# sebasv/lp

Measured on NVIDIA B200. Metric: ipm_iterations_per_s, higher is better.
Workload: dtype f64

## Files before the change

### lp_b200/csrc/cholesky.cu

```cuda
#include <nccl.h>

#include <algorithm>
#include <cstring>
#include <mutex>
#include <type_traits>

#include "dist_schedule.hpp"
#include "kernels.hpp"
#include "panel_factor.cuh"

namespace lpb {

namespace {

constexpr int NB = 128;
constexpr int LDS = NB + 1;
constexpr int TRSM_ROWS = 64;

__global__ void __launch_bounds__(512)
potf2_kernel(double* __restrict__ Mat, int64_t ldm, int k0, int nb, int* __restrict__ info) {
  extern __shared__ double S[];
  double* diag = S + NB * LDS;
  const int tx = threadIdx.x, ty = threadIdx.y, tid = ty * 32 + tx;
  double* blk = Mat + (int64_t)k0 * ldm + k0;
  for (int i = ty; i < nb; i += 16)
    for (int k = tx; k <= i; k += 32) S[i * LDS + k] = blk[(int64_t)i * ldm + k];
  __syncthreads();

  for (int j = 0; j < nb; ++j) {
    const double ajj = S[j * LDS + j];
    if (!(ajj > 0.0) || !isfinite(ajj)) {
      if (tid == 0 && *info == 0) *info = k0 + j + 1;
      for (int i = j + tid; i < nb; i += 512) diag[i] = __longlong_as_double(0x7ff8000000000000ll);
      break;
    }
    const double d = sqrt(ajj);
    if (tid == 0) diag[j] = d;
    if (tid < nb - j - 1) S[(j + 1 + tid) * LDS + j] /= d;
    __syncthreads();
    for (int i = j + 1 + ty; i < nb; i += 16) {
      const double lij = S[i * LDS + j];
      for (int k = j + 1 + tx; k <= i; k += 32) S[i * LDS + k] -= lij * S[k * LDS + j];
    }
    __syncthreads();
  }
  __syncthreads();
  for (int i = ty; i < nb; i += 16)
    for (int k = tx; k <= i; k += 32) blk[(int64_t)i * ldm + k] = (k == i) ? diag[i] : S[i * LDS + k];
}

constexpr int SB = 16;
constexpr int NSB = NB / SB;
constexpr int XDP = SB + 1;
constexpr int TWP = 9;

__device__ __forceinline__ void complete_block_inverse(double* S, const double* rdiag, double* Tw, int tid) {
  const int lane = tid & 31, warp = tid >> 5;
  const int b = warp >> 1, h = warp & 1;
  const int ii = lane & 15, cg = lane >> 4;
  double* tw = Tw + warp * SB * TWP;
  for (int d = 1; d < NSB; ++d) {
    if (b < NSB - d) {
      const int j = b, i = b + d;
      const int ccb = 8 * h + 4 * cg;
      double acc[4] = {0.0, 0.0, 0.0, 0.0};
      const double* lrow = S + (i * SB + ii) * LDS;
#pragma unroll
      for (int l = 0; l < SB; ++l) {
        const double lv = lrow[j * SB + l];
#pragma unroll
        for (int e = 0; e < 4; ++e) {
          const int cc = ccb + e;
          const double up = S[(j * SB + cc) * LDS + j * SB + l];
          const double xv = (l > cc) ? up : ((l == cc) ? rdiag[j * SB + cc] : 0.0);
          acc[e] += lv * xv;
        }
      }
      for (int k = j + 1; k < i; ++k) {
#pragma unroll
        for (int l = 0; l < SB; ++l) {
          const double lv = lrow[k * SB + l];
#pragma unroll
          for (int e = 0; e < 4; ++e) acc[e] += lv * S[(j * SB + ccb + e) * LDS + k * SB + l];
        }
      }
#pragma unroll
      for (int e = 0; e < 4; ++e) tw[ii * TWP + 4 * cg + e] = acc[e];
      __syncwarp();
      double o[4] = {0.0, 0.0, 0.0, 0.0};
#pragma unroll
// ... 1295 lines not shown
int set_smem(K kern, size_t bytes) {
  LPB_CUDA(cudaFuncSetAttribute(kern, cudaFuncAttributeMaxDynamicSharedMemorySize, (int)bytes));
  return LPB_OK;
}

constexpr size_t kPotf2Smem = (size_t)(NB * LDS + NB) * sizeof(double);
constexpr size_t kPotf2InvSmem = (size_t)(NB * LDS + NB + 2 * SB * XDP + 16 * SB * TWP + panel_factor_scratch(XDP)) * sizeof(double);
constexpr size_t kTrsmSmem = (size_t)((NB + TRSM_ROWS) * LDS) * sizeof(double);
constexpr size_t kTrsvSmem = (size_t)(NB * LDS + NB + 2 * NB) * sizeof(double);

int configure_once() {
  static PerDeviceOnce once;
  return once.run([](int) -> int {
  LPB_TRY(set_smem(potf2_kernel, kPotf2Smem));
  LPB_TRY(set_smem(potf2_inv_kernel, kPotf2InvSmem));
  LPB_TRY(set_smem(trsm_kernel, kTrsmSmem));
  LPB_TRY(set_smem(trsm_blocked_kernel, kTrsmBlockedSmem));
  LPB_TRY(set_smem(trsm_dmma_blocked_kernel, kTrsmDmmaSmem));
  LPB_TRY(set_smem(trsv_diag_kernel<false, 1>, kTrsvSmem));
  LPB_TRY(set_smem(trsv_diag_kernel<false, 2>, kTrsvSmem));
  LPB_TRY(set_smem(trsv_diag_kernel<true, 1>, kTrsvSmem));
  LPB_TRY(set_smem(trsv_diag_kernel<true, 2>, kTrsvSmem));
  return LPB_OK;
  });
}

#define LPB_KCHECK(lc)             \
  do {                             \
    (lc).launches++;               \
    LPB_CUDA(cudaGetLastError());  \
  } while (0)

}

struct CholWs {
  int64_t nblk, ldy, off_y, off_flags, off_wt, off_xt, total;
  explicit CholWs(int64_t m) {
    nblk = ceil_div(m, NB);
    ldy = round_up(m, 2);
    off_y = nblk * NB * NB;
    off_flags = off_y + 2 * ldy;
    off_wt = off_flags + round_up(nblk, 2);
    off_xt = off_wt + nblk * 2 * NB * 2;
    total = off_xt + nblk * 2 * NB * 2;
  }
};

static int ensure_chol_ws(LaunchCtx& lc, int64_t m) {
  const int64_t need = CholWs(m).total;
  if (lc.chol_ws_cap >= need) return LPB_OK;
  if (lc.chol_ws) cudaFree(lc.chol_ws);
  lc.chol_ws = nullptr;
  lc.chol_ws_cap = 0;
  lc.linv_valid_m = -1;
  void* p = nullptr;
  LPB_CUDA(cudaMalloc(&p, sizeof(double) * (size_t)need));
  LPB_CUDA(cudaMemsetAsync(p, 0, sizeof(double) * (size_t)need, lc.stream));
  lc.chol_ws = static_cast<double*>(p);
  lc.chol_ws_cap = need;
  return LPB_OK;
}

static int finish_factor(LaunchCtx& lc, int64_t m, double* Mat, int64_t ldm) {
  if (lc.potf2_impl == 1) {
    lc.linv_valid_m = -1;
    lc.linv_mat = nullptr;
    return LPB_OK;
  }
  if (!lc.linv_full) {
    static PerDeviceOnce once;
    LPB_TRY(once.run([](int) -> int { return set_smem(linv_complete_kernel, kLinvCompleteSmem); }));
    linv_complete_kernel<<<(unsigned)ceil_div(m, NB), dim3(32, 16), kLinvCompleteSmem, lc.stream>>>(Mat, ldm, m, lc.chol_ws);
    LPB_KCHECK(lc);
    lc.linv_full = true;
  }
  lc.linv_valid_m = m;
  lc.linv_mat = Mat;
  return LPB_OK;
}

static int k_potrf_dist(LaunchCtx& lc, int64_t m, double* Mat, int64_t ldm);
static int k_potrf_dist2(LaunchCtx& lc, int64_t m, double* Mat, int64_t ldm);

static int k_potrf_lookahead(LaunchCtx& lc, int64_t m, double* Mat, int64_t ldm) {
  if (!lc.side_stream) {
    int lo = 0, hi = 0;
    LPB_CUDA(cudaDeviceGetStreamPriorityRange(&lo, &hi));
    LPB_CUDA(cudaStreamCreateWithPriority(&lc.side_stream, cudaStreamNonBlocking, hi));
    for (int e = 0; e < 2; ++e) {
      LPB_CUDA(cudaEventCreateWithFlags(&lc.ev_col[e], cudaEventDisableTiming));
      LPB_CUDA(cudaEventCreateWithFlags(&lc.ev_pan[e], cudaEventDisableTiming));
    }
  }
  const int T = (int)ceil_div(m, NB);
  lc.linv_full = false;
  auto nb_of = [&](int k) { return (int)((m - (int64_t)k * NB) < NB ? (m - (int64_t)k * NB) : NB); };
  auto potf2 = [&](int k, cudaStream_t st) -> int {
    potf2_inv_kernel<<<1, dim3(32, 16), kPotf2InvSmem, st>>>(Mat, ldm, k * NB, nb_of(k), lc.info_dev,
                                                             lc.chol_ws + (int64_t)k * NB * NB, 0);
    LPB_KCHECK(lc);
    return LPB_OK;
  };
  auto trsm = [&](int k) -> int {
    const int64_t rem = m - (int64_t)k * NB - nb_of(k);
    if (rem <= 0) return LPB_OK;
    trsm_dmma_blocked_kernel<<<(unsigned)ceil_div(rem, TBR), 256, kTrsmDmmaSmem, lc.stream>>>(
        Mat, ldm, k * NB, (int)m, lc.chol_ws + (int64_t)k * NB * NB);
    LPB_KCHECK(lc);
    return LPB_OK;
  };
  LPB_TRY(potf2(0, lc.stream));
  LPB_TRY(trsm(0));
  const int saved_cap = lc.update_grid_cap;
  int rc = LPB_OK;
  for (int k = 0; k + 1 < T && rc == LPB_OK; ++k) {
    const int64_t k0 = (int64_t)k * NB;
    cudaEvent_t ec = lc.ev_col[k & 1], ep = lc.ev_pan[k & 1];
    rc = k_trailing_update_part(lc, m, Mat, ldm, k0, NB, k + 1, 1, 1, 0);
    if (rc != LPB_OK) break;
    LPB_CUDA(cudaEventRecord(ec, lc.stream));
    LPB_CUDA(cudaStreamWaitEvent(lc.side_stream, ec, 0));
    rc = potf2(k + 1, lc.side_stream);
    if (rc != LPB_OK) break;
    LPB_CUDA(cudaEventRecord(ep, lc.side_stream));
    lc.update_grid_cap = kNumSMs - 1;
    rc = k_trailing_update_part(lc, m, Mat, ldm, k0, NB, k + 2, 0, 1, 0);
    lc.update_grid_cap = saved_cap;
    if (rc != LPB_OK) break;
    LPB_CUDA(cudaStreamWaitEvent(lc.stream, ep, 0));
    rc = trsm(k + 1);
  }
  lc.update_grid_cap = saved_cap;
  LPB_TRY(rc);
  return finish_factor(lc, m, Mat, ldm);
}

int k_potrf(LaunchCtx& lc, int64_t m, double* Mat, int64_t ldm, int syrk_impl) {
  LPB_TRY(configure_once());
  LPB_TRY(ensure_chol_ws(lc, m));
  if (lc.ws_m != m) {
    const CholWs ws(m);
    LPB_CUDA(cudaMemsetAsync(lc.chol_ws + ws.off_flags, 0, sizeof(double) * (size_t)(ws.total - ws.off_flags), lc.stream));
    lc.ws_m = m;
  }
  LPB_CUDA(cudaMemsetAsync(lc.info_dev, 0, sizeof(int), lc.stream));
  const bool dmma_update = lc.update_impl == 0 || lc.update_impl == 2 || lc.update_impl == 6;
  if (lc.world > 1 && lc.nccl_comm && lc.potrf_dist && syrk_impl == 0 && lc.trsm_impl == 0 && dmma_update &&
      lc.potf2_impl == 0 && m > NB && !(ldm & 1) && !(reinterpret_cast<uintptr_t>(Mat) & 15))
    return lc.potrf_dist == 2 ? k_potrf_dist2(lc, m, Mat, ldm) : k_potrf_dist(lc, m, Mat, ldm);
  if (lc.potrf_lookahead && syrk_impl == 0 && lc.trsm_impl == 0 && dmma_update && lc.potf2_impl == 0 &&
      !lc.sync_each_launch && m > 2 * NB && !(ldm & 1) && !(reinterpret_cast<uintptr_t>(Mat) & 15))
    return k_potrf_lookahead(lc, m, Mat, ldm);
  const int full_inverse = lc.trsm_impl == 2 ? 1 : 0;
  lc.linv_full = full_inverse != 0;
  for (int64_t k0 = 0; k0 < m; k0 += NB) {
    const int nb = (int)((m - k0) < NB ? (m - k0) : NB);
    const int64_t rem = m - k0 - nb;
    double* linv = lc.chol_ws + (k0 / NB) * NB * NB;
    if (lc.potf2_impl == 1)
      potf2_kernel<<<1, dim3(32, 16), kPotf2Smem, lc.stream>>>(Mat, ldm, (int)k0, nb, lc.info_dev);
    else
      potf2_inv_kernel<<<1, dim3(32, 16), kPotf2InvSmem, lc.stream>>>(Mat, ldm, (int)k0, nb, lc.info_dev, linv,
                                                                      full_inverse);
    LPB_KCHECK(lc);
    if (lc.sync_each_launch) LPB_CUDA(cudaStreamSynchronize(lc.stream));
    if (rem > 0) {
      if (syrk_impl == 1 || lc.trsm_impl == 1) {
        trsm_kernel<<<(unsigned)ceil_div(rem, TRSM_ROWS), dim3(32, 8), kTrsmSmem, lc.stream>>>(Mat, ldm, (int)k0, nb,
                                                                                               (int)m);
        LPB_KCHECK(lc);
      } else if (lc.trsm_impl == 2) {
        LPB_TRY(k_trsm_dmma(lc, m, Mat, ldm, k0, linv));
      } else if (lc.trsm_impl == 3 || (ldm & 1) || (reinterpret_cast<uintptr_t>(Mat) & 15)) {
        trsm_blocked_kernel<<<(unsigned)ceil_div(rem, TBR), 256, kTrsmBlockedSmem, lc.stream>>>(Mat, ldm, (int)k0,
                                                                                               (int)m, linv);
        LPB_KCHECK(lc);
      } else {
        trsm_dmma_blocked_kernel<<<(unsigned)ceil_div(rem, TBR), 256, kTrsmDmmaSmem, lc.stream>>>(Mat, ldm, (int)k0,
                                                                                                 (int)m, linv);
        LPB_KCHECK(lc);
      }
      if (lc.sync_each_launch) LPB_CUDA(cudaStreamSynchronize(lc.stream));
      if (syrk_impl == 1 || lc.update_impl == 1)
        LPB_TRY(k_trailing_update_simple(lc, m, Mat, ldm, k0, nb));
      else
        LPB_TRY(k_trailing_update_dmma(lc, m, Mat, ldm, k0, nb));
      if (lc.sync_each_launch) LPB_CUDA(cudaStreamSynchronize(lc.stream));
    }
  }
  return finish_factor(lc, m, Mat, ldm);
}

static int ensure_dist_streams(LaunchCtx& lc) {
  if (!lc.side_stream) {
    int lo = 0, hi = 0;
    LPB_CUDA(cudaDeviceGetStreamPriorityRange(&lo, &hi));
    LPB_CUDA(cudaStreamCreateWithPriority(&lc.side_stream, cudaStreamNonBlocking, hi));
    for (int e = 0; e < 2; ++e) {
      LPB_CUDA(cudaEventCreateWithFlags(&lc.ev_col[e], cudaEventDisableTiming));
      LPB_CUDA(cudaEventCreateWithFlags(&lc.ev_pan[e], cudaEventDisableTiming));
    }
  }
  for (int e = 0; e < 4; ++e)
    if (!lc.ev_dist[e]) LPB_CUDA(cudaEventCreateWithFlags(&lc.ev_dist[e], cudaEventDisableTiming));
  return LPB_OK;
}

constexpr int kPushCtasPerPeer = 4;
constexpr int kRingHeaderDoubles = 128;
struct PeerPush {
  double* dst[LaunchCtx::kMaxPeers - 1];
  unsigned long long* flag[LaunchCtx::kMaxPeers - 1];
  int n;
};
__global__ void __launch_bounds__(256)
peer_push_kernel(const double* __restrict__ src, int64_t count2, PeerPush pp, unsigned long long value,
                 unsigned* __restrict__ counter) {
  const int peer = blockIdx.x / kPushCtasPerPeer, part = blockIdx.x % kPushCtasPerPeer;
  const double2* s = reinterpret_cast<const double2*>(src);
  double2* d = reinterpret_cast<double2*>(pp.dst[peer]);
  for (int64_t e = part * 256 + threadIdx.x; e < count2; e += kPushCtasPerPeer * 256) d[e] = s[e];
  __threadfence_system();
  __syncthreads();
  if (threadIdx.x == 0) {
    const unsigned done = atomicAdd(counter, 1u);
    if (done == gridDim.x - 1) {
      *counter = 0;
      __threadfence_system();
      for (int g = 0; g < pp.n; ++g)
        asm volatile("st.release.sys.global.u64 [%0], %1;" ::"l"(pp.flag[g]), "l"(value) : "memory");
    }
  }
}
__global__ void wait_flag_kernel(const unsigned long long* __restrict__ flag, unsigned long long value,
                                 unsigned long long* __restrict__ fault) {
  if (threadIdx.x != 0) return;
  unsigned long long t0, t1, v;
  asm volatile("mov.u64 %0, %%globaltimer;" : "=l"(t0));
  for (;;) {
    asm volatile("ld.acquire.sys.global.u64 %0, [%1];" : "=l"(v) : "l"(flag) : "memory");
    if (v >= value) return;
    __nanosleep(100);
    asm volatile("mov.u64 %0, %%globaltimer;" : "=l"(t1));
    if (t1 - t0 > 10000000000ull) {
      if (fault) atomicExch(fault, 1ull);
      return;
    }
    if (fault && *reinterpret_cast<volatile unsigned long long*>(fault) != 0ull) return;
  }
}

static int64_t dist_slot_doubles(int64_t m) { return 3 * (int64_t)NB * NB + round_up(m, NB) * NB; }

struct ProcessRing {
  std::mutex mu;
  double* base = nullptr;
  int64_t slot_doubles = 0;
  int slots = 0, world = 0, rank = -1;
  double* peer[LaunchCtx::kMaxPeers] = {};
  bool mapped = false;
  const LaunchCtx* owner = nullptr;
  uint32_t epoch = 0;
};
static ProcessRing g_ring;

static void ring_free_locked() {
  for (int g = 0; g < LaunchCtx::kMaxPeers; ++g) {
    if (g_ring.peer[g] && g_ring.peer[g] != g_ring.base) cudaIpcCloseMemHandle(g_ring.peer[g]);
    g_ring.peer[g] = nullptr;
  }
  if (g_ring.base) cudaFree(g_ring.base);
  g_ring.base = nullptr;
  g_ring.slots = 0;
  g_ring.slot_doubles = 0;
  g_ring.mapped = false;
}

static void ring_attach_locked(LaunchCtx& lc) {
  lc.ring_base = g_ring.base;
  lc.ring_slots = g_ring.slots;
  lc.ring_slot_doubles = g_ring.slot_doubles;
  for (int g = 0; g < LaunchCtx::kMaxPeers; ++g) lc.peer_base[g] = g_ring.peer[g];
  lc.peer_mapped = g_ring.mapped;
  lc.peer_ready = g_ring.mapped;
  g_ring.owner = &lc;
// ... 438 lines not shown
```

### lp_b200/csrc/common.cuh

```cuda
#pragma once
#include <cuda_runtime.h>
#include <cstdint>
#include <cstdio>
#include <cstring>
#include <mutex>

#include "../../include/lpb200.h"

namespace lpb {

void set_last_error(const char* fmt, ...);
const char* get_last_error();

#define LPB_CUDA(call)                                                                         \
  do {                                                                                         \
    cudaError_t e__ = (call);                                                                  \
    if (e__ != cudaSuccess) {                                                                  \
      ::lpb::set_last_error("%s:%d %s -> %s", __FILE__, __LINE__, #call, cudaGetErrorString(e__)); \
      return LPB_ERR_CUDA;                                                                     \
    }                                                                                          \
  } while (0)

#define LPB_TRY(call)              \
  do {                             \
    int rc__ = (call);             \
    if (rc__ != LPB_OK) return rc__; \
  } while (0)

constexpr int kNumSMs = 148;

constexpr int kMaxDevices = 64;
struct PerDeviceOnce {
  std::mutex mu;
  bool done[kMaxDevices] = {};
  template <class F>
  int run(F&& f) {
    int dev = 0;
    LPB_CUDA(cudaGetDevice(&dev));
    if (dev < 0 || dev >= kMaxDevices) return f(dev);
    std::lock_guard<std::mutex> g(mu);
    if (done[dev]) return LPB_OK;
    const int rc = f(dev);
    if (rc == LPB_OK) done[dev] = true;
    return rc;
  }
};

inline int64_t round_up(int64_t v, int64_t a) { return (v + a - 1) / a * a; }
inline int64_t ceil_div(int64_t a, int64_t b) { return (a + b - 1) / b; }

constexpr int kMaxRedVals = 8;
constexpr int kMaxRedBlocks = 1024;
enum RedOp : int { kRedSum = 0, kRedMin = 1 };

struct LaunchCtx {
  cudaStream_t stream = nullptr;
  int64_t launches = 0;
  double* red_partials = nullptr;
  double* red_out = nullptr;
  double* red_host = nullptr;
  unsigned long long* fault_dev = nullptr;
  double* gemv_partials = nullptr;
  int64_t gemv_partials_cap = 0;
  double* chol_ws = nullptr;
  int64_t chol_ws_cap = 0;
  int64_t ws_m = -1;
  int64_t linv_valid_m = -1;
  const double* linv_mat = nullptr;
  bool linv_full = false;
  int solve_epoch = 0;
  int solve_impl = 0;
  int sync_each_launch = 0;
  int syrk_flush_blocks = 32;
  int syrk_tail_split = 1;
  double* syrk_ws = nullptr;
  int64_t syrk_ws_cap = 0;
  int syrk_chain = 0;
  int potf2_impl = 0;
  int trsm_impl = 0, update_impl = 0;
  int solve_grid_cap = 0;
  void* nccl_comm = nullptr;
  int rank = 0, world = 1;
  int potrf_dist = 2;
  double* panel_buf = nullptr;
  int64_t panel_buf_cap = 0;
  int potrf_lookahead = 1;
  cudaStream_t side_stream = nullptr;
  cudaEvent_t ev_col[2] = {nullptr, nullptr}, ev_pan[2] = {nullptr, nullptr};
  bool launch_on_side = false;
  cudaEvent_t ev_dist[4] = {nullptr, nullptr, nullptr, nullptr};
  double* panel_slot[2] = {nullptr, nullptr};
  int64_t panel_slot_cap = 0;
  static constexpr int kMaxPeers = 8;
  double* ring_base = nullptr;
  int64_t ring_slot_doubles = 0;
  int ring_slots = 0;
  double* peer_base[kMaxPeers] = {};
  bool peer_mapped = false;
  bool peer_ready = false;
  uint32_t dist_epoch = 0;
  int update_grid_cap = 0;
  int* info_dev = nullptr;
  int* info_host = nullptr;
};

}
```

### lp_b200/csrc/dist_schedule.hpp

```cpp
#pragma once
#include <cmath>

#if defined(__CUDACC__)
#define LPB_SCHED_HD __host__ __device__
#else
#define LPB_SCHED_HD
#endif

namespace lpb {

struct OwnedCols {
  int G, f, n;
  LPB_SCHED_HD int before(int l) const { return l * (n - f) - G * (l * (l - 1) / 2); }
  LPB_SCHED_HD int count() const {
    if (f >= n) return 0;
    const int nown = (n - f + G - 1) / G;
    return before(nown);
  }
  LPB_SCHED_HD void decode(int t, int* ti, int* tj) const {
    const double a = 0.5 * G, b = (n - f) + 0.5 * G;
    const double disc = b * b - 4.0 * a * t;
    int l = static_cast<int>((b - sqrt(disc > 0.0 ? disc : 0.0)) / (2.0 * a));
    if (l < 0) l = 0;
    while (l > 0 && before(l) > t) --l;
    while (before(l + 1) <= t) ++l;
    *tj = f + l * G;
    *ti = *tj + (t - before(l));
  }
  static LPB_SCHED_HD OwnedCols make(int G, int rank, int tile0, int ntr) {
    OwnedCols o;
    o.G = G;
    o.f = ((rank - tile0) % G + G) % G;
    o.n = ntr;
    return o;
  }
};

template <class Ops>
int potrf_dist_schedule(int T, int G, int me, Ops& ops) {
  int pending = -1;
  for (int k = 0; k < T; ++k) {
    const int owner = k % G;
    int rc;
    if (owner == me && (rc = ops.factor_panel(k)) != 0) return rc;
    if ((rc = ops.broadcast(k, owner)) != 0) return rc;
    if (owner != me && (rc = ops.store_panel(k)) != 0) return rc;
    if (pending >= 0) {
      if ((rc = ops.update_owned(pending, pending + 2)) != 0) return rc;
      pending = -1;
    }
    if (k + 1 < T) {
      if ((k + 1) % G == me) {
        if ((rc = ops.update_column(k, k + 1)) != 0) return rc;
        pending = k;
      } else if ((rc = ops.update_owned(k, k + 1)) != 0) {
        return rc;
      }
    }
  }
  return 0;
}

enum { kEvSmall = 0, kEvPotf2 = 2, kNumDistEvents = 4 };

template <class Ops>
int potrf_dist_schedule2(int T, int G, int me, Ops& ops) {
#define LPB_S2(call)            \
  do {                          \
    const int rc__ = (call);    \
    if (rc__ != 0) return rc__; \
  } while (0)
  int pending = -1;
  for (int k = 0; k < T; ++k) {
    const int owner = k % G;
    if (owner == me) {
      if (k == 0)
        LPB_S2(ops.potf2(0, 0));
      else
        LPB_S2(ops.wait(kEvPotf2 + (k & 1), 0));
      LPB_S2(ops.trsm(k));
    }
    if (k + 1 < T) {
      LPB_S2(ops.bcast_small(k, owner));
      LPB_S2(ops.record(kEvSmall + (k & 1), 0));
    }
    LPB_S2(ops.bcast_large(k, owner));
    if (pending >= 0) {
      LPB_S2(ops.update_owned(pending, pending + 2));
      if (pending % G != me) LPB_S2(ops.unpack(pending));
      pending = -1;
    }
    if (k + 1 < T && (k + 1) % G == me) {
      LPB_S2(ops.wait(kEvSmall + (k & 1), 1));
      LPB_S2(ops.update_diag(k, k + 1, 1));
      LPB_S2(ops.potf2(k + 1, 1));
      LPB_S2(ops.record(kEvPotf2 + ((k + 1) & 1), 1));
      LPB_S2(ops.update_col_below(k, k + 1));
      pending = k;
    } else {
      if (k + 1 < T) LPB_S2(ops.update_owned(k, k + 1));
// ... 10 lines not shown
```

### lp_b200/csrc/dmma_gemm.cu

```cuda
#include <cuda.h>

#include "dist_schedule.hpp"
#include "kernels.hpp"

namespace lpb {

namespace {

constexpr int BM = 128, BN = 128, BK = 16;
constexpr int kStages = 5;
constexpr int kLead = 3;
constexpr int kFlushBlocks = 128;
constexpr int kConsumerWarps = 8;
constexpr int kThreads = kConsumerWarps * 32;
constexpr uint32_t kTileBytes = BM * BK * 8;
constexpr uint32_t kDBytes = BK * 8;
constexpr uint32_t kSmemA = 0;
constexpr uint32_t kSmemB = kSmemA + kStages * kTileBytes;
constexpr uint32_t kSmemD = kSmemB + kStages * kTileBytes;
constexpr uint32_t kSmemBar = kSmemD + kStages * kDBytes;
constexpr uint32_t kSmemTotal = kSmemBar + 2 * kStages * 8;
constexpr uint32_t kSmemAlloc = kSmemTotal + 1024;

template <int MODE, int VAR>
// ... 440 lines not shown
        }
      }
    }
    if (VAR & 2) __syncthreads();
  }
}

__global__ void __launch_bounds__(256)
syrk_tail_fixup_kernel(double* __restrict__ C, int64_t ldc, int m_total, int ntr, TailSplit ts) {
  int ti, tj;
  band_decode(ts.n_full + blockIdx.x, ntr, &ti, &tj);
  const double* w = ts.ws + static_cast<int64_t>(blockIdx.x) * ts.nsplit * (BM * BN);
  for (int e = threadIdx.x; e < BM * BN / 2; e += 256) {
    const int r = ti * BM + (e >> 6), c = tj * BN + 2 * (e & 63);
    if (r >= m_total || c >= m_total) continue;
    double2 sum = make_double2(0.0, 0.0);
    for (int p = 0; p < ts.nsplit; ++p) {
      const double2 v = *reinterpret_cast<const double2*>(w + static_cast<int64_t>(p) * (BM * BN) + 2 * e);
      sum.x += v.x;
      sum.y += v.y;
    }
    *reinterpret_cast<double2*>(C + static_cast<int64_t>(r) * ldc + c) = sum;
  }
}

typedef CUresult (*EncodeTiledFn)(CUtensorMap*, CUtensorMapDataType, cuuint32_t, void*, const cuuint64_t*,
                                  const cuuint64_t*, const cuuint32_t*, const cuuint32_t*, CUtensorMapInterleave,
                                  CUtensorMapSwizzle, CUtensorMapL2promotion, CUtensorMapFloatOOBfill);

int get_encode_fn(EncodeTiledFn* out) {
  static std::mutex mu;
  static EncodeTiledFn fn = nullptr;
  std::lock_guard<std::mutex> g(mu);
  if (!fn) {
    void* p = nullptr;
    cudaDriverEntryPointQueryResult q;
    LPB_CUDA(cudaGetDriverEntryPoint("cuTensorMapEncodeTiled", &p, cudaEnableDefault, &q));
    if (q != cudaDriverEntryPointSuccess || !p) {
      set_last_error("cuTensorMapEncodeTiled not available from the driver");
      return LPB_ERR_CUDA;
    }
    fn = reinterpret_cast<EncodeTiledFn>(p);
  }
  *out = fn;
  return LPB_OK;
}

int make_tmap(CUtensorMap* tm, const double* base, uint64_t rows, uint64_t cols, uint64_t ld, uint32_t box_rows,
              uint32_t box_cols, bool swizzle) {
  EncodeTiledFn fn;
  LPB_TRY(get_encode_fn(&fn));
  const cuuint64_t dims[2] = {cols, rows};
  const cuuint64_t strides[1] = {ld * sizeof(double)};
  const cuuint32_t box[2] = {box_cols, box_rows};
  const cuuint32_t estr[2] = {1, 1};
  const CUresult r = fn(tm, CU_TENSOR_MAP_DATA_TYPE_FLOAT64, 2, const_cast<double*>(base), dims, strides, box, estr,
                        CU_TENSOR_MAP_INTERLEAVE_NONE,
                        swizzle ? CU_TENSOR_MAP_SWIZZLE_128B : CU_TENSOR_MAP_SWIZZLE_NONE,
                        CU_TENSOR_MAP_L2_PROMOTION_L2_256B, CU_TENSOR_MAP_FLOAT_OOB_FILL_NONE);
  if (r != CUDA_SUCCESS) {
    set_last_error("cuTensorMapEncodeTiled failed (%d): base=%p rows=%llu cols=%llu ld=%llu", (int)r, (const void*)base,
                   (unsigned long long)rows, (unsigned long long)cols, (unsigned long long)ld);
    return LPB_ERR_CUDA;
  }
  return LPB_OK;
}

template <int MODE, bool SCALE, int VAR = 0>
int launch_dmma(LaunchCtx& lc, const CUtensorMap& tmA, const CUtensorMap& tmB, double* C, int64_t ldc, int m_total,
                int tile0, int ntr, int k_begin, int nkb, int col_origin, int shape = SHAPE_TRI,
                OwnedCols own = OwnedCols{1, 0, 0}, int p_row0 = -1, TailSplit ts = TailSplit{0, 1, nullptr}) {
  static PerDeviceOnce once;
  auto kern = syrk_dmma_kernel<MODE, SCALE, VAR>;
  LPB_TRY(once.run([&](int) -> int {
    LPB_CUDA(cudaFuncSetAttribute(kern, cudaFuncAttributeMaxDynamicSharedMemorySize, (int)Plan<MODE, VAR>::kAlloc));
    return LPB_OK;
  }));
  const int ntiles = (MODE == MODE_TRSM || shape == SHAPE_COL) ? ntr
                     : (shape == SHAPE_COLB ? ntr - 1 : (shape == SHAPE_OWNED ? own.count() : ntr * (ntr + 1) / 2));
  if (ntiles <= 0) return LPB_OK;
  if (ts.nsplit <= 1) ts = TailSplit{ntiles, 1, nullptr};
  int grid = ntiles < kNumSMs ? ntiles : kNumSMs;
  if (MODE == MODE_UPDATE && lc.update_grid_cap > 0 && grid > lc.update_grid_cap) grid = lc.update_grid_cap;
  cudaStream_t st = lc.launch_on_side ? lc.side_stream : lc.stream;
  kern<<<grid, kThreads, Plan<MODE, VAR>::kAlloc, st>>>(tmA, tmB, C, ldc, m_total, tile0, ntr, k_begin, nkb, col_origin, shape, own,
                                           p_row0, ts);
  lc.launches++;
  LPB_CUDA(cudaGetLastError());
  return LPB_OK;
}

}

int k_syrk_dmma(LaunchCtx& lc, int64_t m, int64_t n, const double* A, int64_t lda, const double* d, double* Cmat,
                int64_t ldc) {
  if ((lda & 1) || (ldc & 1) || (reinterpret_cast<uintptr_t>(A) & 15) || (reinterpret_cast<uintptr_t>(Cmat) & 15) ||
      (d && (reinterpret_cast<uintptr_t>(d) & 15))) {
    set_last_error("syrk_dmma: A, d, M must be 16-byte aligned with even leading dimensions");
    return LPB_ERR_BAD_ARGUMENT;
  }
  if (m <= 0 || n <= 0) return LPB_OK;
  CUtensorMap tmA, tmD;
  LPB_TRY(make_tmap(&tmA, A, (uint64_t)m, (uint64_t)n, (uint64_t)lda, BM, BK, true));
  if (d)
    LPB_TRY(make_tmap(&tmD, d, 1, (uint64_t)n, (uint64_t)round_up(n, 2), 1, BK, false));
  else
    tmD = tmA;
  const int ntr = (int)ceil_div(m, BM);
  const int nkb = (int)ceil_div(n, BK);
  if (lc.syrk_chain) {
    if (d) return launch_dmma<MODE_SYRK, true, 16>(lc, tmA, tmD, Cmat, ldc, (int)m, 0, ntr, 0, nkb, 0);
    return launch_dmma<MODE_SYRK, false, 16>(lc, tmA, tmD, Cmat, ldc, (int)m, 0, ntr, 0, nkb, 0);
  }
  const int fb = lc.syrk_flush_blocks;
  TailSplit ts{0, 1, nullptr};
  const int ntiles = ntr * (ntr + 1) / 2;
  const int rem = ntiles % kNumSMs;
  if (lc.syrk_tail_split && ntiles > kNumSMs && rem > 0 && 4 * rem <= 3 * kNumSMs && nkb >= 64 && !(m & 1)) {
    int best_s = 1;
    double best = 1.0;
    for (int sp = 2; sp <= 8; ++sp) {
      const double len = (double)ceil_div((int64_t)rem * sp, (int64_t)kNumSMs) / sp + 0.01 * sp;
      if (len < best - 1e-9) {
        best = len;
        best_s = sp;
      }
    }
    if (best_s > 1) {
      const int64_t need = (int64_t)rem * best_s * BM * BN;
      if (lc.syrk_ws_cap < need) {
        if (lc.syrk_ws) LPB_CUDA(cudaFree(lc.syrk_ws));
        lc.syrk_ws = nullptr;
        lc.syrk_ws_cap = 0;
        void* p = nullptr;
        LPB_CUDA(cudaMalloc(&p, sizeof(double) * (size_t)need));
        lc.syrk_ws = static_cast<double*>(p);
        lc.syrk_ws_cap = need;
      }
      ts = TailSplit{ntiles - rem, best_s, lc.syrk_ws};
    }
  }
  if (ts.nsplit > 1) {
    if (d)
      LPB_TRY((launch_dmma<MODE_SYRK, true, 32>(lc, tmA, tmD, Cmat, ldc, (int)m, 0, ntr, 0, nkb, fb, SHAPE_TRI, OwnedCols{1, 0, 0}, -1, ts)));
    else
      LPB_TRY((launch_dmma<MODE_SYRK, false, 32>(lc, tmA, tmD, Cmat, ldc, (int)m, 0, ntr, 0, nkb, fb, SHAPE_TRI, OwnedCols{1, 0, 0}, -1, ts)));
  } else if (d) {
    LPB_TRY((launch_dmma<MODE_SYRK, true>(lc, tmA, tmD, Cmat, ldc, (int)m, 0, ntr, 0, nkb, fb)));
  } else {
    LPB_TRY((launch_dmma<MODE_SYRK, false>(lc, tmA, tmD, Cmat, ldc, (int)m, 0, ntr, 0, nkb, fb)));
  }
  if (ts.nsplit > 1) {
    syrk_tail_fixup_kernel<<<rem, 256, 0, lc.stream>>>(Cmat, ldc, (int)m, ntr, ts);
    lc.launches++;
    LPB_CUDA(cudaGetLastError());
  }
  return LPB_OK;
}

int k_trailing_update_dmma(LaunchCtx& lc, int64_t m, double* Mat, int64_t ldm, int64_t k0, int64_t kb) {
  const int64_t row0 = k0 + kb;
  if (row0 >= m) return LPB_OK;
  if ((row0 % BM) || (kb % BK) || (ldm & 1) || (reinterpret_cast<uintptr_t>(Mat) & 15)) {
    set_last_error("trailing_update_dmma: panel origin must be a multiple of %d, width a multiple of %d", BM, BK);
    return LPB_ERR_BAD_ARGUMENT;
  }
  CUtensorMap tm;
  LPB_TRY(make_tmap(&tm, Mat, (uint64_t)m, (uint64_t)m, (uint64_t)ldm, BM, BK, true));
  const int ntr = (int)ceil_div(m - row0, BM);
  if (lc.update_impl == 2)
    return launch_dmma<MODE_UPDATE, false, 1>(lc, tm, tm, Mat, ldm, (int)m, (int)(row0 / BM), ntr, (int)k0,
                                              (int)(kb / BK), 0);
  if (lc.update_impl == 3)
    return launch_dmma<MODE_UPDATE, false, 2>(lc, tm, tm, Mat, ldm, (int)m, (int)(row0 / BM), ntr, (int)k0,
                                              (int)(kb / BK), 0);
  if (lc.update_impl == 4)
    return launch_dmma<MODE_UPDATE, false, 4>(lc, tm, tm, Mat, ldm, (int)m, (int)(row0 / BM), ntr, (int)k0,
                                              (int)(kb / BK), 0);
  if (lc.update_impl == 5)
    return launch_dmma<MODE_UPDATE, false, 6>(lc, tm, tm, Mat, ldm, (int)m, (int)(row0 / BM), ntr, (int)k0,
                                              (int)(kb / BK), 0);
  return launch_dmma<MODE_UPDATE, false>(lc, tm, tm, Mat, ldm, (int)m, (int)(row0 / BM), ntr, (int)k0, (int)(kb / BK),
                                         0);
}

int k_trailing_update_part(LaunchCtx& lc, int64_t m, double* Mat, int64_t ldm, int64_t k0, int64_t kb, int tile0,
                           int single_col, int own_mod, int own_rem, const double* packed, int64_t packed_rows) {
  int ntr = (int)ceil_div(m, BM) - tile0;
  if (ntr <= 0) return LPB_OK;
  if ((kb % BK) || (ldm & 1) || (reinterpret_cast<uintptr_t>(Mat) & 15) || (int64_t)tile0 * BM < k0 + kb) {
    set_last_error("trailing_update_part: bad panel / tile origin");
    return LPB_ERR_BAD_ARGUMENT;
  }
  CUtensorMap tm, tmc;
  int k_begin = (int)k0, p_row0 = -1;
  LPB_TRY(make_tmap(&tmc, Mat, (uint64_t)m, (uint64_t)m, (uint64_t)ldm, BM, BK, true));
  if (packed) {
    LPB_TRY(make_tmap(&tm, packed, (uint64_t)packed_rows, (uint64_t)BN, (uint64_t)BN, BM, BK, true));
    k_begin = 0;
    p_row0 = (int)k0;
  } else {
    tm = tmc;
  }
  int shape = SHAPE_TRI;
  if (single_col == 1) shape = SHAPE_COL;
  if (single_col == 2) {
    shape = SHAPE_COL;
    ntr = 1;
  }
  if (single_col == 3) shape = SHAPE_COLB;
  if (!single_col && own_mod > 1) shape = SHAPE_OWNED;
  const OwnedCols own = shape == SHAPE_OWNED ? OwnedCols::make(own_mod, own_rem, tile0, ntr) : OwnedCols{1, 0, 0};
  if (lc.update_impl == 2)
    return launch_dmma<MODE_UPDATE, false, 1>(lc, tm, tm, Mat, ldm, (int)m, tile0, ntr, k_begin, (int)(kb / BK), 0, shape,
                                              own, p_row0);
  if (lc.update_impl == 6)
    return launch_dmma<MODE_UPDATE, false, 8>(lc, tm, tmc, Mat, ldm, (int)m, tile0, ntr, k_begin, (int)(kb / BK), 0,
                                              shape, own, p_row0);
  return launch_dmma<MODE_UPDATE, false>(lc, tm, tm, Mat, ldm, (int)m, tile0, ntr, k_begin, (int)(kb / BK), 0, shape, own,
                                         p_row0);
}

int k_trsm_dmma(LaunchCtx& lc, int64_t m, double* Mat, int64_t ldm, int64_t k0, const double* Linv) {
  const int64_t row0 = k0 + BN;
  if (row0 >= m) return LPB_OK;
  if ((row0 % BM) || (ldm & 1) || (reinterpret_cast<uintptr_t>(Mat) & 15) || (reinterpret_cast<uintptr_t>(Linv) & 15)) {
    set_last_error("trsm_dmma: panel origin must be a multiple of %d", BM);
    return LPB_ERR_BAD_ARGUMENT;
  }
  CUtensorMap tm, tl;
  LPB_TRY(make_tmap(&tm, Mat, (uint64_t)m, (uint64_t)m, (uint64_t)ldm, BM, BK, true));
  LPB_TRY(make_tmap(&tl, Linv, (uint64_t)BN, (uint64_t)BN, (uint64_t)BN, BN, BK, true));
  const int ntr = (int)ceil_div(m - row0, BM);
  return launch_dmma<MODE_TRSM, false>(lc, tm, tl, Mat, ldm, (int)m, (int)(row0 / BM), ntr, (int)k0, BN / BK, (int)k0);
}

__global__ void __launch_bounds__(256)
dmma_peak_kernel(double* out, int iters, double a0, double b0) {
  double c[32][2];
#pragma unroll
  for (int i = 0; i < 32; ++i) c[i][0] = c[i][1] = threadIdx.x * 1e-3 + i;
  const double a = a0 + threadIdx.x * 1e-9, b = b0;
  for (int it = 0; it < iters; ++it) {
#pragma unroll
    for (int i = 0; i < 32; ++i) dmma884(c[i][0], c[i][1], a, b);
  }
  double s = 0.0;
#pragma unroll
  for (int i = 0; i < 32; ++i) s += c[i][0] + c[i][1];
  if (s == 12345.678) out[0] = s;
}

int k_dmma_peak(LaunchCtx& lc, double seconds, double* tflops) {
  if (seconds < 0.05) seconds = 0.05;
  if (seconds > 2.0) seconds = 2.0;
  const int iters = 4000;
  const double flop_per_launch = 2.0 * 256 * 32 * iters * 8.0 * kNumSMs;
  cudaEvent_t e0, e1;
  LPB_CUDA(cudaEventCreate(&e0));
  LPB_CUDA(cudaEventCreate(&e1));
  auto run = [&](int launches, float* ms) -> int {
    LPB_CUDA(cudaEventRecord(e0, lc.stream));
    for (int i = 0; i < launches; ++i) dmma_peak_kernel<<<kNumSMs, 256, 0, lc.stream>>>(lc.red_partials, iters, 1.0000001, 1e-9);
    LPB_CUDA(cudaEventRecord(e1, lc.stream));
    LPB_CUDA(cudaEventSynchronize(e1));
    LPB_CUDA(cudaEventElapsedTime(ms, e0, e1));
    lc.launches += launches;
    return LPB_OK;
  };
  float ms = 0.f;
  int rc = run(4, &ms);
  if (rc == LPB_OK) {
    int launches = (int)(seconds * 1e3 / (ms / 4.0 > 1e-3 ? ms / 4.0 : 1e-3));
    if (launches < 8) launches = 8;
    if (launches > 4000) launches = 4000;
    rc = run(launches, &ms);
    if (rc == LPB_OK && tflops) *tflops = flop_per_launch * launches / (ms * 1e-3) * 1e-12;
  }
  cudaEventDestroy(e0);
  cudaEventDestroy(e1);
  return rc;
}

template <bool ACCUM>
__global__ void __launch_bounds__(256)
syrk_simple_kernel(int m_total, int row_origin, int k_begin, int k_end, const double* __restrict__ A, int64_t lda,
                   const double* __restrict__ d, double* __restrict__ C, int64_t ldc) {
  __shared__ double sa[16][65], sb[16][65];
  const int bi = blockIdx.y, bj = blockIdx.x;
  if (bj > bi) return;
  const int tx = threadIdx.x & 15, ty = threadIdx.x >> 4, tid = threadIdx.x;
  double acc[4][4];
#pragma unroll
  for (int i = 0; i < 4; ++i)
#pragma unroll
    for (int j = 0; j < 4; ++j) acc[i][j] = 0.0;
  for (int k0 = k_begin; k0 < k_end; k0 += 16) {
#pragma unroll
    for (int e = 0; e < 4; ++e) {
      const int idx = tid + e * 256, r = idx >> 4, k = idx & 15;
      const int gk = k0 + k, gi = row_origin + bi * 64 + r, gj = row_origin + bj * 64 + r;
      const bool kin = gk < k_end;
      sa[k][r] = (kin && gi < m_total) ? A[(int64_t)gi * lda + gk] : 0.0;
// ... 54 lines not shown
```

### lp_b200/csrc/kernels.hpp

```cpp
#pragma once
#include "common.cuh"

namespace lpb {

struct RedSpec {
  int nvals = 0;
  int nblocks[kMaxRedVals] = {0};
  int op[kMaxRedVals] = {0};
};
int reduce_finalize(LaunchCtx& lc, const RedSpec& spec);
int fetch_scalars(LaunchCtx& lc, int nvals);

int k_fill(LaunchCtx& lc, double* p, int64_t n, double v);
int k_copy(LaunchCtx& lc, double* dst, const double* src, int64_t n);
int k_dinv(LaunchCtx& lc, int64_t n, const double* x, const double* z, double* dinv);

int k_rhat(LaunchCtx& lc, int64_t n, int mode, double eta, double gm, double a2, double s, const double* x,
           const double* z, const double* rD, const double* dx, const double* dz, double* xs, double* r1);

int k_assemble_delta_n(LaunchCtx& lc, int64_t n, double d_tau, const double* u, const double* p, const double* xs,
                       const double* x, const double* z, double* dx, double* dz, int val_base, int* nblocks);
int k_assemble_delta_m(LaunchCtx& lc, int64_t m, double d_tau, const double* v, const double* q, double* dy);
int k_step(LaunchCtx& lc, int64_t n, double alpha, int clamp, double* x, const double* dx);
int k_extract_x(LaunchCtx& lc, int64_t n, double tau, const double* x, const double* c, double* xo, int val,
                int* nblocks);

int k_resid_p(LaunchCtx& lc, int64_t m, double tau, const double* b, const double* t, const double* y, double* rP,
              int val_base, int* nblocks);
int k_sym_fwd_rhs(LaunchCtx& lc, int64_t m, double eta, const double* rP, const double* b, const double* t0,
                  const double* t1, double* rhs0, double* rhs1, int with_pq);
int k_refine_rhs(LaunchCtx& lc, int64_t m, double eta, const double* rP, const double* b, const double* au,
                 const double* ap, double* rho0, double* rho1, int with_pq);
int k_add_inplace(LaunchCtx& lc, int64_t count, const double* x, double* y);
int k_dots_m(LaunchCtx& lc, int64_t m, const double* b, const double* v, const double* q, int with_pq, int val_base,
             int* nblocks);

int k_gemv_n(LaunchCtx& lc, int64_t m, int64_t n, const double* A, int64_t lda, const double* dinv, const double* w0,
             const double* w1, double* t0, double* t1, int nrhs);
int k_gemv_t_partials(LaunchCtx& lc, int64_t m, int64_t n, const double* A, int64_t lda, const double* v0,
                      const double* v1, int nrhs, int* nchunks);
struct TailCols {
  int64_t nd;
  const int* col_row;
  const double* col_val;
  const double* v0;
  const double* v1;
};
int k_gemv_t_raw(LaunchCtx& lc, int64_t n, int nchunks, int nrhs, double* out0, double* out1);
int k_resid_d(LaunchCtx& lc, int64_t n, int nchunks, double tau, const double* c, const double* z, const double* x,
              double* rD, int val_base, int* nblocks, const TailCols* tail = nullptr);
int k_sym_back(LaunchCtx& lc, int64_t n, int nchunks, int with_pq, const double* dinv, const double* r1,
               const double* c, double* u, double* p, int val_base, int* nblocks, const TailCols* tail = nullptr);

int k_syrk_dmma(LaunchCtx& lc, int64_t m, int64_t n, const double* A, int64_t lda, const double* d, double* Cmat,
                int64_t ldc);
int k_trailing_update_dmma(LaunchCtx& lc, int64_t m, double* Mat, int64_t ldm, int64_t k0, int64_t kb);
int k_trailing_update_part(LaunchCtx& lc, int64_t m, double* Mat, int64_t ldm, int64_t k0, int64_t kb, int tile0,
                           int single_col, int own_mod, int own_rem, const double* packed = nullptr,
                           int64_t packed_rows = 0);
int k_trsm_dmma(LaunchCtx& lc, int64_t m, double* Mat, int64_t ldm, int64_t k0, const double* Linv);
int k_dmma_peak(LaunchCtx& lc, double seconds, double* tflops);
int k_syrk_simple(LaunchCtx& lc, int64_t m, int64_t n, const double* A, int64_t lda, const double* d, double* Cmat,
                  int64_t ldc);
int k_trailing_update_simple(LaunchCtx& lc, int64_t m, double* Mat, int64_t ldm, int64_t k0, int64_t kb);

int k_potrf(LaunchCtx& lc, int64_t m, double* Mat, int64_t ldm, int syrk_impl);
int k_potrf_dist_reserve(LaunchCtx& lc, int64_t m);
int k_peer_export(LaunchCtx& lc, int64_t m, unsigned char* handle_out, int* state_out);
int k_peer_import(LaunchCtx& lc, const unsigned char* handles, int world);
void k_peer_release(LaunchCtx& lc);
void k_peer_abandon(LaunchCtx& lc);
void k_peer_free_process();
int k_potrs(LaunchCtx& lc, int64_t m, const double* L, int64_t ldm, double* B, int nrhs, bool use_linv);

int k_fill_normal(LaunchCtx& lc, double* A, int64_t rows, int64_t cols, int64_t lda, int64_t row0, int64_t col0,
                  uint64_t seed);
int k_fill_vec(LaunchCtx& lc, double* v, int64_t count, int64_t idx0, uint64_t seed, int kind, double lo, double hi,
               int64_t neg_below);
int k_slack_identity(LaunchCtx& lc, double* A, int64_t rows, int64_t cols, int64_t lda, int64_t col0, int64_t n0);
int k_add_vec(LaunchCtx& lc, double* out, const double* a, const double* b, int64_t count, int64_t count_b);
int k_col_structure(LaunchCtx& lc, const double* A, int64_t m, int64_t n, int64_t lda, int* nnz, int* row, double* val);
int k_diag_add(LaunchCtx& lc, int64_t m, double* M, int64_t ldm, const int* col, const double* val, const double* dinv);
int k_diag_shift(LaunchCtx& lc, int64_t m, double* M, int64_t ldm, double delta);
int k_slack_add(LaunchCtx& lc, int64_t m, const int* col, const double* val, const double* dinv, const double* w0,
                const double* w1, double* t0, double* t1, int nrhs);
int64_t tri_packed_doubles(int64_t m);
int k_tri_pack(LaunchCtx& lc, double* M, int64_t ldm, int64_t m, double* buf, bool pack);
int k_diff(LaunchCtx& lc, const double* a, const double* b, int64_t rows, int64_t cols, int64_t ld, int lower_only,
           unsigned long long* out_dev3);
int k_checksum(LaunchCtx& lc, const double* v, int64_t rows, int64_t cols, int64_t ld, int lower_only,
               unsigned long long* out_dev);

}
```

### lp_b200/csrc/lpb_api.cu

```cuda
#include <nccl.h>

#include <algorithm>
#include <chrono>
#include <cmath>
#include <cstdlib>
#include <mutex>
#include <new>
#include <string>
#include <vector>

#include "ipm_driver.hpp"
#include "kernels.hpp"

namespace lpb {
int64_t gemv_t_partials_doubles(int64_t m, int64_t n);
int batched_launch(int64_t batch, int m, int n, const double* dA, const double* db, const double* dc,
                   const lpb_options& o, double* dx, double* dfun, int64_t* dit, int32_t* dst, cudaStream_t stream);
}

using namespace lpb;

enum Phase { PH_SYRK = 0, PH_POTRF, PH_SOLVE, PH_SWEEP, PH_VEC, PH_COMM, PH_COUNT };

struct PhaseRec {
// ... 1286 lines not shown
  *out = c->prof;
  return LPB_OK;
}

int64_t lpb_launch_count(lpb_ctx* c) { return c ? c->lc.launches : 0; }

int lpb_measure_dmma_peak(lpb_ctx* c, double seconds, double* tflops_out) {
  if (!c || !tflops_out) return LPB_ERR_BAD_ARGUMENT;
  return k_dmma_peak(c->lc, seconds, tflops_out);
}

int lpb_set_option(lpb_ctx* c, const char* key, int64_t value) {
  if (!c || !key) return LPB_ERR_BAD_ARGUMENT;
  const std::string k(key);
  if (k == "syrk_impl") {
    if (value != 0 && value != 1) return LPB_ERR_BAD_ARGUMENT;
    c->syrk_impl = (int)value;
    return LPB_OK;
  }
  if (k == "solve_impl") {
    if (value < 0 || value > 3) return LPB_ERR_BAD_ARGUMENT;
    c->lc.solve_impl = (int)value;
    return LPB_OK;
  }
  if (k == "trsm_impl" || k == "update_impl") {
    if (value < 0 || value > 6) return LPB_ERR_BAD_ARGUMENT;
    (k == "trsm_impl" ? c->lc.trsm_impl : c->lc.update_impl) = (int)value;
    return LPB_OK;
  }
  if (k == "syrk_tail_split") {
    c->lc.syrk_tail_split = value != 0;
    return LPB_OK;
  }
  if (k == "syrk_chain") {
    c->lc.syrk_chain = value != 0;
    return LPB_OK;
  }
  if (k == "peer_panels") {
    if (value > 0 && !c->lc.peer_mapped) return LPB_ERR_BAD_ARGUMENT;
    if (value < 0)
      k_peer_abandon(c->lc);
    else
      c->lc.peer_ready = value != 0;
    return LPB_OK;
  }
  if (k == "syrk_flush_blocks") {
    if (value < 32 || value > (1 << 20) || (value & (value - 1))) return LPB_ERR_BAD_ARGUMENT;
    c->lc.syrk_flush_blocks = (int)value;
    return LPB_OK;
  }
  if (k == "potf2_impl") {
    if (value < 0 || value > 1) return LPB_ERR_BAD_ARGUMENT;
    c->lc.potf2_impl = (int)value;
    if (value == 1) c->lc.trsm_impl = 1;
    return LPB_OK;
  }
  if (k == "solve_grid_cap") {
    if (value < 0) return LPB_ERR_BAD_ARGUMENT;
    c->lc.solve_grid_cap = (int)value;
    return LPB_OK;
  }
  if (k == "refine") {
    if (value < 0 || value > 4) return LPB_ERR_BAD_ARGUMENT;
    c->refine = (int)value;
    return LPB_OK;
  }
  if (k == "refine_max") {
    if (value < 0 || value > 8) return LPB_ERR_BAD_ARGUMENT;
    c->refine_max = (int)value;
    return LPB_OK;
  }
  if (k == "regularize") {
    c->regularize = value != 0;
    return LPB_OK;
  }
  if (k == "structure") {
    c->use_structure = value != 0;
    return c->has_problem ? analyze_structure(c) : LPB_OK;
  }
  if (k == "potrf_lookahead") {
    c->lc.potrf_lookahead = value != 0;
    return LPB_OK;
  }
  if (k == "packed_allreduce") {
    c->packed_allreduce = value != 0;
    return LPB_OK;
  }
  if (k == "potrf_dist") {
    if (value < 0 || value > 2) return LPB_ERR_BAD_ARGUMENT;
    c->lc.potrf_dist = (int)value;
    return LPB_OK;
  }
  if (k == "potrf_verify") {
    c->potrf_verify = (int)value;
    return LPB_OK;
  }
  if (k == "sync_each_launch") {
    c->lc.sync_each_launch = (int)value;
    return LPB_OK;
  }
  if (k == "check_replicas") {
    c->check_replicas = value != 0;
    return LPB_OK;
  }
  if (k == "profile") {
    c->profile = value != 0;
    return LPB_OK;
  }
  set_last_error("unknown option '%s'", key);
  return LPB_ERR_BAD_ARGUMENT;
}

}
```

Before: 4.005.

## Add grouped left-looking Cholesky schedule overlapping far trailing updates with panel groups

New measurement: 4.105 (median of 6 runs). 2.5% higher.

```diff
diff --git a/lp_b200/csrc/cholesky.cu b/lp_b200/csrc/cholesky.cu
--- a/lp_b200/csrc/cholesky.cu
+++ b/lp_b200/csrc/cholesky.cu
@@ -6,6 +6,7 @@
 #include <type_traits>
 
 #include "dist_schedule.hpp"
+#include "group_schedule.hpp"
 #include "kernels.hpp"
 #include "panel_factor.cuh"
 
@@ -1467,7 +1468,7 @@
 static int k_potrf_dist(LaunchCtx& lc, int64_t m, double* Mat, int64_t ldm);
 static int k_potrf_dist2(LaunchCtx& lc, int64_t m, double* Mat, int64_t ldm);
 
-static int k_potrf_lookahead(LaunchCtx& lc, int64_t m, double* Mat, int64_t ldm) {
+static int ensure_side_stream(LaunchCtx& lc) {
   if (!lc.side_stream) {
     int lo = 0, hi = 0;
     LPB_CUDA(cudaDeviceGetStreamPriorityRange(&lo, &hi));
@@ -1477,6 +1478,11 @@
       LPB_CUDA(cudaEventCreateWithFlags(&lc.ev_pan[e], cudaEventDisableTiming));
     }
   }
+  return LPB_OK;
+}
+
+static int k_potrf_lookahead(LaunchCtx& lc, int64_t m, double* Mat, int64_t ldm) {
+  LPB_TRY(ensure_side_stream(lc));
   const int T = (int)ceil_div(m, NB);
   lc.linv_full = false;
   auto nb_of = [&](int k) { return (int)((m - (int64_t)k * NB) < NB ? (m - (int64_t)k * NB) : NB); };
@@ -1520,6 +1526,56 @@
   return finish_factor(lc, m, Mat, ldm);
 }
 
+constexpr int64_t kGroupedMinM = 8192;
+
+static int k_potrf_grouped(LaunchCtx& lc, int64_t m, double* Mat, int64_t ldm, int g) {
+  LPB_TRY(ensure_side_stream(lc));
+  lc.linv_full = false;
+  const int T = (int)ceil_div(m, NB);
+  struct Ops {
+    LaunchCtx& lc;
+    int64_t m;
+    double* Mat;
+    int64_t ldm;
+    cudaEvent_t ev[kNumGroupEvents];
+    cudaStream_t st(int side) const { return side ? lc.side_stream : lc.stream; }
+    int nb(int k) const { return (int)((m - (int64_t)k * NB) < NB ? (m - (int64_t)k * NB) : NB); }
+    int potf2(int k) {
+      potf2_inv_kernel<<<1, dim3(32, 16), kPotf2InvSmem, lc.side_stream>>>(Mat, ldm, k * NB, nb(k), lc.info_dev,
+                                                                         lc.chol_ws + (int64_t)k * NB * NB, 0);
+      LPB_KCHECK(lc);
+      return LPB_OK;
+    }
+    int trsm(int k) {
+      const int64_t rem = m - (int64_t)k * NB - nb(k);
+      if (rem <= 0) return LPB_OK;
+      trsm_dmma_blocked_kernel<<<(unsigned)ceil_div(rem, TBR), 256, kTrsmDmmaSmem, lc.side_stream>>>(
+          Mat, ldm, k * NB, (int)m, lc.chol_ws + (int64_t)k * NB * NB);
+      LPB_KCHECK(lc);
+      return LPB_OK;
+    }
+    int update(int p0, int np, int col0, int ncol, int side) {
+      lc.launch_on_side = side != 0;
+      lc.update_tiles_per_cta = side ? 0 : 1;
+      const int rc = k_trailing_update_cols(lc, m, Mat, ldm, (int64_t)p0 * NB, (int64_t)np * NB, col0, ncol);
+      lc.launch_on_side = false;
+      lc.update_tiles_per_cta = 0;
+      return rc;
+    }
+    int record(int e, int side) {
+      LPB_CUDA(cudaEventRecord(ev[e], st(side)));
+      return LPB_OK;
+    }
+    int wait(int e, int side) {
+      LPB_CUDA(cudaStreamWaitEvent(st(side), ev[e], 0));
+      return LPB_OK;
+    }
+  } ops{lc, m, Mat, ldm, {lc.ev_col[0], lc.ev_col[1], lc.ev_pan[0], lc.ev_pan[1]}};
+  static_assert(kNumGroupEvents == 4, "k_potrf_grouped maps the schedule's events onto ev_col / ev_pan");
+  LPB_TRY(potrf_group_schedule(T, g, g, ops));
+  return finish_factor(lc, m, Mat, ldm);
+}
+
 int k_potrf(LaunchCtx& lc, int64_t m, double* Mat, int64_t ldm, int syrk_impl) {
   LPB_TRY(configure_once());
   LPB_TRY(ensure_chol_ws(lc, m));
@@ -1534,8 +1590,11 @@
       lc.potf2_impl == 0 && m > NB && !(ldm & 1) && !(reinterpret_cast<uintptr_t>(Mat) & 15))
     return lc.potrf_dist == 2 ? k_potrf_dist2(lc, m, Mat, ldm) : k_potrf_dist(lc, m, Mat, ldm);
   if (lc.potrf_lookahead && syrk_impl == 0 && lc.trsm_impl == 0 && dmma_update && lc.potf2_impl == 0 &&
-      !lc.sync_each_launch && m > 2 * NB && !(ldm & 1) && !(reinterpret_cast<uintptr_t>(Mat) & 15))
+      !lc.sync_each_launch && m > 2 * NB && !(ldm & 1) && !(reinterpret_cast<uintptr_t>(Mat) & 15)) {
+    const int g = lc.potrf_group >= 0 ? lc.potrf_group : (m < kGroupedMinM ? 0 : (m < 16384 ? 4 : 6));
+    if (g > 0 && lc.update_impl == 0) return k_potrf_grouped(lc, m, Mat, ldm, g);
     return k_potrf_lookahead(lc, m, Mat, ldm);
+  }
   const int full_inverse = lc.trsm_impl == 2 ? 1 : 0;
   lc.linv_full = full_inverse != 0;
   for (int64_t k0 = 0; k0 < m; k0 += NB) {
@@ -1577,15 +1636,7 @@
 }
 
 static int ensure_dist_streams(LaunchCtx& lc) {
-  if (!lc.side_stream) {
-    int lo = 0, hi = 0;
-    LPB_CUDA(cudaDeviceGetStreamPriorityRange(&lo, &hi));
-    LPB_CUDA(cudaStreamCreateWithPriority(&lc.side_stream, cudaStreamNonBlocking, hi));
-    for (int e = 0; e < 2; ++e) {
-      LPB_CUDA(cudaEventCreateWithFlags(&lc.ev_col[e], cudaEventDisableTiming));
-      LPB_CUDA(cudaEventCreateWithFlags(&lc.ev_pan[e], cudaEventDisableTiming));
-    }
-  }
+  LPB_TRY(ensure_side_stream(lc));
   for (int e = 0; e < 4; ++e)
     if (!lc.ev_dist[e]) LPB_CUDA(cudaEventCreateWithFlags(&lc.ev_dist[e], cudaEventDisableTiming));
   return LPB_OK;
diff --git a/lp_b200/csrc/common.cuh b/lp_b200/csrc/common.cuh
--- a/lp_b200/csrc/common.cuh
+++ b/lp_b200/csrc/common.cuh
@@ -100,6 +100,8 @@
   bool peer_ready = false;
   uint32_t dist_epoch = 0;
   int update_grid_cap = 0;
+  int update_tiles_per_cta = 0;
+  int potrf_group = -1;
   int* info_dev = nullptr;
   int* info_host = nullptr;
 };
diff --git a/lp_b200/csrc/dist_schedule.hpp b/lp_b200/csrc/dist_schedule.hpp
--- a/lp_b200/csrc/dist_schedule.hpp
+++ b/lp_b200/csrc/dist_schedule.hpp
@@ -11,11 +11,12 @@
 
 struct OwnedCols {
   int G, f, n;
+  int cols = 1 << 30;
   LPB_SCHED_HD int before(int l) const { return l * (n - f) - G * (l * (l - 1) / 2); }
   LPB_SCHED_HD int count() const {
     if (f >= n) return 0;
     const int nown = (n - f + G - 1) / G;
-    return before(nown);
+    return before(nown < cols ? nown : cols);
   }
   LPB_SCHED_HD void decode(int t, int* ti, int* tj) const {
     const double a = 0.5 * G, b = (n - f) + 0.5 * G;
diff --git a/lp_b200/csrc/dmma_gemm.cu b/lp_b200/csrc/dmma_gemm.cu
--- a/lp_b200/csrc/dmma_gemm.cu
+++ b/lp_b200/csrc/dmma_gemm.cu
@@ -546,6 +546,7 @@
   if (ts.nsplit <= 1) ts = TailSplit{ntiles, 1, nullptr};
   int grid = ntiles < kNumSMs ? ntiles : kNumSMs;
   if (MODE == MODE_UPDATE && lc.update_grid_cap > 0 && grid > lc.update_grid_cap) grid = lc.update_grid_cap;
+  if (MODE == MODE_UPDATE && lc.update_tiles_per_cta > 0) grid = (int)ceil_div(ntiles, lc.update_tiles_per_cta);
   cudaStream_t st = lc.launch_on_side ? lc.side_stream : lc.stream;
   kern<<<grid, kThreads, Plan<MODE, VAR>::kAlloc, st>>>(tmA, tmB, C, ldc, m_total, tile0, ntr, k_begin, nkb, col_origin, shape, own,
                                            p_row0, ts);
@@ -683,6 +684,24 @@
                                               shape, own, p_row0);
   return launch_dmma<MODE_UPDATE, false>(lc, tm, tm, Mat, ldm, (int)m, tile0, ntr, k_begin, (int)(kb / BK), 0, shape, own,
                                          p_row0);
+}
+
+int k_trailing_update_cols(LaunchCtx& lc, int64_t m, double* Mat, int64_t ldm, int64_t k0, int64_t kb, int tile0,
+                           int ncol) {
+  const int ntr = (int)ceil_div(m, BM) - tile0;
+  if (ntr <= 0) return LPB_OK;
+  if (kb <= 0 || (kb % BK) || (ldm & 1) || (reinterpret_cast<uintptr_t>(Mat) & 15) || (int64_t)tile0 * BM < k0 + kb) {
+    set_last_error("trailing_update_cols: bad panel / tile origin");
+    return LPB_ERR_BAD_ARGUMENT;
+  }
+  CUtensorMap tm;
+  LPB_TRY(make_tmap(&tm, Mat, (uint64_t)m, (uint64_t)m, (uint64_t)ldm, BM, BK, true));
+  if (ncol <= 0 || ncol >= ntr)
+    return launch_dmma<MODE_UPDATE, false>(lc, tm, tm, Mat, ldm, (int)m, tile0, ntr, (int)k0, (int)(kb / BK), 0);
+  OwnedCols cols{1, 0, ntr};
+  cols.cols = ncol;
+  return launch_dmma<MODE_UPDATE, false>(lc, tm, tm, Mat, ldm, (int)m, tile0, ntr, (int)k0, (int)(kb / BK), 0,
+                                         SHAPE_OWNED, cols);
 }
 
 int k_trsm_dmma(LaunchCtx& lc, int64_t m, double* Mat, int64_t ldm, int64_t k0, const double* Linv) {
diff --git a/lp_b200/csrc/group_schedule.hpp b/lp_b200/csrc/group_schedule.hpp
--- /dev/null
+++ b/lp_b200/csrc/group_schedule.hpp
@@ -0,0 +1,46 @@
+#pragma once
+
+namespace lpb {
+
+enum { kEvGroupIn = 0, kEvGroupPanels = 1, kEvGroupFar = 2, kEvGroupOut = 3, kNumGroupEvents = 4 };
+
+template <class Ops>
+int potrf_group_schedule(int T, int g, int W, Ops& ops) {
+#define LPB_G(call)             \
+  do {                          \
+    const int rc__ = (call);    \
+    if (rc__ != 0) return rc__; \
+  } while (0)
+  LPB_G(ops.record(kEvGroupIn, 0));
+  LPB_G(ops.wait(kEvGroupIn, 1));
+  LPB_G(ops.potf2(0));
+  bool far_pending = false;
+  for (int c0 = 0; c0 < T; c0 += g) {
+    const int c1 = c0 + g < T ? c0 + g : T;
+    for (int p = c0; p < c1; ++p) {
+      LPB_G(ops.trsm(p));
+      if (p + 1 < c1) {
+        LPB_G(ops.update(p, 1, p + 1, c1 - p - 1, 1));
+        LPB_G(ops.potf2(p + 1));
+      }
+    }
+    if (c1 == T) break;
+    LPB_G(ops.record(kEvGroupPanels, 1));
+    const int c2 = c1 + W < T ? c1 + W : T;
+    if (far_pending) LPB_G(ops.wait(kEvGroupFar, 1));
+    LPB_G(ops.update(c0, c1 - c0, c1, c2 - c1, 1));
+    LPB_G(ops.potf2(c1));
+    far_pending = c2 < T;
+    if (far_pending) {
+      LPB_G(ops.wait(kEvGroupPanels, 0));
+      LPB_G(ops.update(c0, c1 - c0, c2, 0, 0));
+      LPB_G(ops.record(kEvGroupFar, 0));
+    }
+  }
+  LPB_G(ops.record(kEvGroupOut, 1));
+  LPB_G(ops.wait(kEvGroupOut, 0));
+#undef LPB_G
+  return 0;
+}
+
+}
diff --git a/lp_b200/csrc/kernels.hpp b/lp_b200/csrc/kernels.hpp
--- a/lp_b200/csrc/kernels.hpp
+++ b/lp_b200/csrc/kernels.hpp
@@ -58,6 +58,8 @@
 int k_trailing_update_part(LaunchCtx& lc, int64_t m, double* Mat, int64_t ldm, int64_t k0, int64_t kb, int tile0,
                            int single_col, int own_mod, int own_rem, const double* packed = nullptr,
                            int64_t packed_rows = 0);
+int k_trailing_update_cols(LaunchCtx& lc, int64_t m, double* Mat, int64_t ldm, int64_t k0, int64_t kb, int tile0,
+                           int ncol);
 int k_trsm_dmma(LaunchCtx& lc, int64_t m, double* Mat, int64_t ldm, int64_t k0, const double* Linv);
 int k_dmma_peak(LaunchCtx& lc, double seconds, double* tflops);
 int k_syrk_simple(LaunchCtx& lc, int64_t m, int64_t n, const double* A, int64_t lda, const double* d, double* Cmat,
diff --git a/lp_b200/csrc/lpb_api.cu b/lp_b200/csrc/lpb_api.cu
--- a/lp_b200/csrc/lpb_api.cu
+++ b/lp_b200/csrc/lpb_api.cu
@@ -1392,6 +1392,11 @@
     c->lc.potrf_lookahead = value != 0;
     return LPB_OK;
   }
+  if (k == "potrf_group") {
+    if (value < -1 || value > 16) return LPB_ERR_BAD_ARGUMENT;
+    c->lc.potrf_group = (int)value;
+    return LPB_OK;
+  }
   if (k == "packed_allreduce") {
     c->packed_allreduce = value != 0;
     return LPB_OK;
```
